# 3dlg-hcvc/tricolo

Measured on AMD Instinct MI355X. Metric: trimodal training samples/sec (32^3 voxel + 6-view), higher is better.
Workload: dtype f16 (f16 activation storage + f16 MFMA operands, fp32 accumulate; bf16x3 heads/GRU; within 1e-3 of the fp32 reference)

## Files before the change

tricolo_amd/csrc/bn_pool.hip:

```cpp
#include "common.h"
#include "../../include/tricolo_hip.h"

__global__ void bn_finalize_kernel(const float* __restrict__ partial, int ntiles, int C, const int* __restrict__ count_dev,
                                   int count_host, const float* __restrict__ gamma, const float* __restrict__ beta,
                                   float* running_mean, float* running_var, long long* num_batches_tracked, float momentum,
                                   float eps, float* __restrict__ mean_out, float* __restrict__ invstd_out,
                                   float* __restrict__ scale_out, float* __restrict__ shift_out) {
    __shared__ double ssum[4], ssq[4];
    const int c = blockIdx.x;
    float pg = 0.f, pb = 0.f, prm = 0.f, prv = 0.f;
    int pcount = count_host;
    if (threadIdx.x == 0) {
        pg = gamma[c]; pb = beta[c];
        if (running_mean) { prm = running_mean[c]; prv = running_var[c]; }
        if (count_dev) pcount = *count_dev;
    }
    double s = 0.0, q = 0.0;
#pragma unroll 8
    for (int tIdx = threadIdx.x; tIdx < ntiles; tIdx += 256) {
        s += (double)partial[((size_t)tIdx * 2 + 0) * C + c];
        q += (double)partial[((size_t)tIdx * 2 + 1) * C + c];
    }
#pragma unroll
    for (int o = 32; o > 0; o >>= 1) { s += __shfl_xor(s, o); q += __shfl_xor(q, o); }
// ... 691 lines not shown
    const int tc = threadIdx.x % tpr, tr = threadIdx.x / tpr;
    const int n = *row_count;
    for (int cc = 0; cc < cpt; ++cc) {
        const int c4 = tc + cc * tpr;
        float4 sg = make_float4(0, 0, 0, 0), sgy = make_float4(0, 0, 0, 0);
        if (c4 < C4 && tr < rpp)
#pragma unroll 4
            for (int i = blockIdx.x * rpp + tr; i < n; i += gridDim.x * rpp) {
                const long r = row_pos[i];
                const float4 gv = Act<T>::ld4(g + r * C + c4 * 4), yv = Act<T>::ld4(y + r * C + c4 * 4);
                sg.x += gv.x; sg.y += gv.y; sg.z += gv.z; sg.w += gv.w;
                sgy.x += gv.x * yv.x; sgy.y += gv.y * yv.y; sgy.z += gv.z * yv.z; sgy.w += gv.w * yv.w;
            }
        __syncthreads();
        if (c4 < C4 && tr < rpp) {
            float* p = sh + ((size_t)tr * tpr + tc) * 8;
            p[0] = sg.x; p[1] = sg.y; p[2] = sg.z; p[3] = sg.w; p[4] = sgy.x; p[5] = sgy.y; p[6] = sgy.z; p[7] = sgy.w;
        }
        __syncthreads();
        if (tr == 0 && c4 < C4) {
            float a[8] = {0, 0, 0, 0, 0, 0, 0, 0};
            for (int rr = 0; rr < rpp; ++rr) {
                const float* p = sh + ((size_t)rr * tpr + tc) * 8;
#pragma unroll
                for (int k = 0; k < 8; ++k) a[k] += p[k];
            }
            float* o = partial + (size_t)blockIdx.x * 2 * C;
#pragma unroll
            for (int k = 0; k < 4; ++k) { o[c4 * 4 + k] = a[k]; o[C + c4 * 4 + k] = a[4 + k]; }
        }
    }
}
template <typename T>
__global__ void bn_bwd_apply_rows_kernel(const T* __restrict__ y, const T* g, const float4* __restrict__ c1, const float4* __restrict__ c2,
                                         const float4* __restrict__ c3, T* dy, int C4, const int* __restrict__ row_pos,
                                         const int* __restrict__ row_count) {
    const long total = (long)(*row_count) * C4;
    for (long i = (long)blockIdx.x * blockDim.x + threadIdx.x; i < total; i += (long)gridDim.x * blockDim.x) {
        const int c = (int)(i % C4);
        const long o = ((long)row_pos[i / C4] * C4 + c) * 4;
        const float4 yv = Act<T>::ld4(y + o), gv = Act<T>::ld4(g + o), a = c1[c], b = c2[c], d = c3[c];
        Act<T>::st4(dy + o, make_float4(a.x * gv.x + b.x + d.x * yv.x, a.y * gv.y + b.y + d.y * yv.y, a.z * gv.z + b.z + d.z * yv.z,
                                        a.w * gv.w + b.w + d.w * yv.w));
    }
}
extern "C" size_t tri_bn_bwd_rows_scratch(int C) { return (size_t)BNR_BLOCKS * 2 * C * sizeof(float) + 3 * (size_t)C * sizeof(float); }
extern "C" int tri_bn_bwd_rows(const void* y, const void* g, int C, const int* row_pos, const int* row_count, long max_rows, const float* gamma,
                               const float* mean, const float* invstd, void* dy, float* dgamma, float* dbeta, float out_scale, void* scratch,
                               int act_fmt, void* stream) {
    if (C % 4 || !row_pos || !row_count || !scratch) { tri_set_error("tri_bn_bwd_rows: C % 4, row list and scratch required"); return TRI_ERR_ARG; }
    hipStream_t st = (hipStream_t)stream;
    float* partial = (float*)scratch;
    float* co = partial + (size_t)BNR_BLOCKS * 2 * C;
    const int C4 = C / 4, tpr = C4 < 256 ? C4 : 256, rpp = 256 / tpr;
    const size_t smem = (size_t)rpp * tpr * 8 * sizeof(float);
    TRI_ACT_DISPATCH(act_fmt, bn_bwd_reduce_rows_kernel<T><<<BNR_BLOCKS, 256, smem, st>>>((const T*)y, (const T*)g, C, row_pos, row_count, partial));
    bn_bwd_finalize_kernel<<<C, 256, 0, st>>>(partial, BNR_BLOCKS, C, row_count, 0, gamma, mean, invstd, dgamma, dbeta, co, co + C, co + 2 * C, out_scale);
    const int grid = ew_grid(max_rows * C4 / 4 + 1);
    TRI_ACT_DISPATCH(act_fmt, bn_bwd_apply_rows_kernel<T><<<grid, 256, 0, st>>>((const T*)y, (const T*)g, (const float4*)co, (const float4*)(co + C),
                                                                                 (const float4*)(co + 2 * C), (T*)dy, C4, row_pos, row_count));
    return tri_check_launch("tri_bn_bwd_rows");
}

extern "C" int tri_bn_bwd_apply_rows(const void* y, const void* g, const float* c1, const float* c2, const float* c3, void* dy, int C,
                                     const int* row_pos, const int* row_count, long max_rows, int act_fmt, void* stream) {
    if (C % 4 || !row_pos || !row_count) { tri_set_error("tri_bn_bwd_apply_rows: C % 4 and a row list required"); return TRI_ERR_ARG; }
    const int C4 = C / 4, grid = ew_grid(max_rows * C4 / 4 + 1);
    TRI_ACT_DISPATCH(act_fmt, bn_bwd_apply_rows_kernel<T><<<grid, 256, 0, (hipStream_t)stream>>>((const T*)y, (const T*)g, (const float4*)c1,
        (const float4*)c2, (const float4*)c3, (T*)dy, C4, row_pos, row_count));
    return tri_check_launch("tri_bn_bwd_apply_rows");
}

template <typename T>
__global__ __launch_bounds__(256) void pool3d_bwd_route_reduce_kernel(const T* __restrict__ y, const float4* __restrict__ scale,
                                                                      const float4* __restrict__ shift, const uint8_t* __restrict__ mask,
                                                                      const T* __restrict__ pooled, const T* __restrict__ dpooled, int B, int D,
                                                                      int C4, T* __restrict__ g, float* __restrict__ partial) {
    __shared__ float sh[256][8];
    const int Do = D >> 1;
    const long total = (long)B * Do * Do * Do * C4;
    const int c = threadIdx.x % C4;
    const float4 s = scale[c], t = shift[c];
    float4 sg = make_float4(0.f, 0.f, 0.f, 0.f), sgy = sg;
    for (unsigned i = blockIdx.x * blockDim.x + threadIdx.x; i < (unsigned)total; i += gridDim.x * blockDim.x) {
        const PoolWin w = pool_window(mask, i / (unsigned)C4, (unsigned)D);
        if (!w.bits) continue;
        const float4 pm = Act<T>::ld4(pooled + (size_t)i * 4), dp = Act<T>::ld4(dpooled + (size_t)i * 4);
        route_window<T>(y, s, t, w, (unsigned)D, (unsigned)C4, (unsigned)c, pm, dp, g, sg, sgy);
    }
    float* p = sh[threadIdx.x];
    p[0] = sg.x; p[1] = sg.y; p[2] = sg.z; p[3] = sg.w; p[4] = sgy.x; p[5] = sgy.y; p[6] = sgy.z; p[7] = sgy.w;
    __syncthreads();
    if ((int)threadIdx.x < C4) {
        float a[8] = {0, 0, 0, 0, 0, 0, 0, 0};
        for (int r = threadIdx.x; r < 256; r += C4)
#pragma unroll
            for (int k = 0; k < 8; ++k) a[k] += sh[r][k];
        float* o = partial + (size_t)blockIdx.x * 2 * C4 * 4;
#pragma unroll
        for (int k = 0; k < 4; ++k) { o[c * 4 + k] = a[k]; o[C4 * 4 + c * 4 + k] = a[4 + k]; }
    }
}
extern "C" int tri_pool3d_bwd_route_reduce_num_blocks(int B, int D, int C) {
    return ew_grid((long)B * (D / 2) * (D / 2) * (D / 2) * (C / 4));
}
extern "C" int tri_pool3d_bwd_route_reduce(const void* y, const float* scale, const float* shift, const uint8_t* mask, const void* pooled,
                                           const void* dpooled, int B, int D, int C, void* g, float* partial, int act_fmt, void* stream) {
    if (C % 4 || C / 4 > 256 || 256 % (C / 4)) { tri_set_error("tri_pool3d_bwd_route_reduce: C / 4 must divide 256"); return TRI_ERR_ARG; }
    if (!pool_args_ok("tri_pool3d_bwd_route_reduce", mask, B, D, C)) return TRI_ERR_ARG;
    const int nblk = tri_pool3d_bwd_route_reduce_num_blocks(B, D, C);
    TRI_ACT_DISPATCH(act_fmt, pool3d_bwd_route_reduce_kernel<T><<<nblk, 256, 0, (hipStream_t)stream>>>(
        (const T*)y, (const float4*)scale, (const float4*)shift, mask, (const T*)pooled, (const T*)dpooled, B, D, C / 4, (T*)g, partial));
    return tri_check_launch("tri_pool3d_bwd_route_reduce");
}

template <typename T>
__global__ void maxpool2d_fwd_kernel(const T* __restrict__ x, int N, int H, int W, int C4, T* __restrict__ out,
                                     uchar4* __restrict__ arg, const float4* __restrict__ scale, const float4* __restrict__ shift) {
    const int Ho = (H + 1) / 2, Wo = (W + 1) / 2;
    const long total = (long)N * Ho * Wo * C4;
    for (long i = (long)blockIdx.x * blockDim.x + threadIdx.x; i < total; i += (long)gridDim.x * blockDim.x) {
        int c = (int)(i % C4);
        long pos = i / C4;
        int ow = (int)(pos % Wo); long r = pos / Wo;
        int oh = (int)(r % Ho); int n = (int)(r / Ho);
        float4 best = make_float4(-INFINITY, -INFINITY, -INFINITY, -INFINITY);
        uchar4 bi = make_uchar4(0, 0, 0, 0);
        float4 s4 = make_float4(1.f, 1.f, 1.f, 1.f), b4 = make_float4(0.f, 0.f, 0.f, 0.f);
        if (scale) { s4 = scale[c]; b4 = shift[c]; }
#pragma unroll
        for (int kh = 0; kh < 3; ++kh) {
            int ih = oh * 2 - 1 + kh;
            if ((unsigned)ih >= (unsigned)H) continue;
#pragma unroll
            for (int kw = 0; kw < 3; ++kw) {
                int iw = ow * 2 - 1 + kw;
                if ((unsigned)iw >= (unsigned)W) continue;
                float4 v = Act<T>::ld4(x + ((((long)n * H + ih) * W + iw) * C4 + c) * 4);
                if (scale) {
                    v.x = fmaxf(__fmaf_rn(v.x, s4.x, b4.x), 0.f); v.y = fmaxf(__fmaf_rn(v.y, s4.y, b4.y), 0.f);
                    v.z = fmaxf(__fmaf_rn(v.z, s4.z, b4.z), 0.f); v.w = fmaxf(__fmaf_rn(v.w, s4.w, b4.w), 0.f);
                }
                unsigned char k = (unsigned char)(kh * 3 + kw);
                if (v.x > best.x) { best.x = v.x; bi.x = k; }
                if (v.y > best.y) { best.y = v.y; bi.y = k; }
                if (v.z > best.z) { best.z = v.z; bi.z = k; }
                if (v.w > best.w) { best.w = v.w; bi.w = k; }
            }
        }
        Act<T>::st4(out + i * 4, best);
        if (arg) arg[i] = bi;
    }
}
template <typename T>
__global__ __launch_bounds__(256) void maxpool2d_fwd8_kernel(const T* __restrict__ x, int N, int H, int W, int C8, T* __restrict__ out,
                                                             uint2* __restrict__ arg, const float* __restrict__ scale, const float* __restrict__ shift) {
    const int Ho = (H + 1) / 2, Wo = (W + 1) / 2;
    constexpr int G = 4;
    const int Hg = (Ho + G - 1) / G;
    const long total = (long)N * Hg * Wo * C8;
    for (long i = (long)blockIdx.x * blockDim.x + threadIdx.x; i < total; i += (long)gridDim.x * blockDim.x) {
        const int c = (int)(i % C8);
        long pos = i / C8;
        const int ow = (int)(pos % Wo); long r = pos / Wo;
        const int og = (int)(r % Hg); const int n = (int)(r / Hg);
        float s8[8], b8[8];
#pragma unroll
        for (int k = 0; k < 8; ++k) { s8[k] = 1.f; b8[k] = 0.f; }
        if (scale) {
#pragma unroll
            for (int k = 0; k < 8; ++k) { s8[k] = scale[c * 8 + k]; b8[k] = shift[c * 8 + k]; }
        }
        bool okw[3];
#pragma unroll
        for (int kw = 0; kw < 3; ++kw) okw[kw] = (unsigned)(ow * 2 - 1 + kw) < (unsigned)W;
        auto load_row = [&](int ih, uint4 (&d)[3]) {
#pragma unroll
            for (int kw = 0; kw < 3; ++kw) {
                d[kw] = make_uint4(0u, 0u, 0u, 0u);
                if ((unsigned)ih < (unsigned)H && okw[kw]) d[kw] = *(const uint4*)(x + ((((long)n * H + ih) * W + ow * 2 - 1 + kw) * C8 + c) * 8);
            }
        };
        uint4 row0[3], row1[3], row2[3];
        const int oh0 = og * G;
        load_row(oh0 * 2 - 1, row0);
#pragma unroll
        for (int g = 0; g < G; ++g) {
            const int oh = oh0 + g;
            if (oh >= Ho) break;
            load_row(oh * 2, row1);
            load_row(oh * 2 + 1, row2);
            float best[8];
            unsigned bi[8];
#pragma unroll
            for (int k = 0; k < 8; ++k) { best[k] = -INFINITY; bi[k] = 0u; }
#pragma unroll
            for (int kh = 0; kh < 3; ++kh) {
                if ((unsigned)(oh * 2 - 1 + kh) >= (unsigned)H) continue;
#pragma unroll
                for (int kw = 0; kw < 3; ++kw) {
                    if (!okw[kw]) continue;
                    const uint4 q = kh == 0 ? row0[kw] : (kh == 1 ? row1[kw] : row2[kw]);
#pragma unroll
                    for (int k = 0; k < 8; ++k) {
                        float e = (float)((const T*)&q)[k];
                        if (scale) e = fmaxf(__fmaf_rn(e, s8[k], b8[k]), 0.f);
                        if (e > best[k]) { best[k] = e; bi[k] = (unsigned)(kh * 3 + kw); }
                    }
                }
            }
            uint4 o;
            T* op = (T*)&o;
#pragma unroll
            for (int k = 0; k < 8; ++k) op[k] = (T)best[k];
            const long oi = (((long)n * Ho + oh) * Wo + ow) * C8 + c;
            *(uint4*)(out + oi * 8) = o;
            if (arg) arg[oi] = make_uint2(bi[0] | (bi[1] << 8) | (bi[2] << 16) | (bi[3] << 24), bi[4] | (bi[5] << 8) | (bi[6] << 16) | (bi[7] << 24));
#pragma unroll
            for (int kw = 0; kw < 3; ++kw) row0[kw] = row2[kw];
        }
    }
}
extern "C" int tri_maxpool2d_fwd(const void* x, int N, int H, int W, int C, void* out, uint8_t* arg, const float* bn_scale,
                                 const float* bn_shift, int act_fmt, void* stream) {
    static int pool8 = -1;
    if (pool8 < 0) pool8 = 1;
    if (pool8 && act_fmt != TRI_FMT_F32 && C % 8 == 0) {
        const long total8 = (long)N * (((H + 1) / 2 + 3) / 4) * ((W + 1) / 2) * (C / 8);
        if (act_fmt == TRI_FMT_F16)
            maxpool2d_fwd8_kernel<f16_t><<<ew_grid(total8), 256, 0, (hipStream_t)stream>>>((const f16_t*)x, N, H, W, C / 8, (f16_t*)out, (uint2*)arg, bn_scale, bn_shift);
        else
            maxpool2d_fwd8_kernel<bf16_t><<<ew_grid(total8), 256, 0, (hipStream_t)stream>>>((const bf16_t*)x, N, H, W, C / 8, (bf16_t*)out, (uint2*)arg, bn_scale, bn_shift);
        return tri_check_launch("tri_maxpool2d_fwd");
    }
    long total = (long)N * ((H + 1) / 2) * ((W + 1) / 2) * (C / 4);
    TRI_ACT_DISPATCH(act_fmt, maxpool2d_fwd_kernel<T><<<ew_grid(total), 256, 0, (hipStream_t)stream>>>((const T*)x, N, H, W, C / 4, (T*)out, (uchar4*)arg,
                                                                                                  (const float4*)bn_scale, (const float4*)bn_shift));
    return tri_check_launch("tri_maxpool2d_fwd");
}

template <typename T>
__global__ void maxpool2d_bwd_kernel(const uchar4* __restrict__ arg, const T* __restrict__ dout, int N, int H, int W, int C4,
                                     T* __restrict__ dx) {
    const int Ho = (H + 1) / 2, Wo = (W + 1) / 2;
    const long total = (long)N * H * W * C4;
    for (long i = (long)blockIdx.x * blockDim.x + threadIdx.x; i < total; i += (long)gridDim.x * blockDim.x) {
        int c = (int)(i % C4);
        long pos = i / C4;
        int w = (int)(pos % W); long r = pos / W;
        int h = (int)(r % H); int n = (int)(r / H);
        float4 acc = make_float4(0.f, 0.f, 0.f, 0.f);
        for (int oh = h / 2; oh <= (h + 1) / 2; ++oh) {
            if (oh >= Ho) continue;
            for (int ow = w / 2; ow <= (w + 1) / 2; ++ow) {
                if (ow >= Wo) continue;
                unsigned char me = (unsigned char)((h - (oh * 2 - 1)) * 3 + (w - (ow * 2 - 1)));
                long o = (((long)n * Ho + oh) * Wo + ow) * C4 + c;
                uchar4 a = arg[o];
                float4 d = Act<T>::ld4(dout + o * 4);
                if (a.x == me) acc.x += d.x;
                if (a.y == me) acc.y += d.y;
                if (a.z == me) acc.z += d.z;
                if (a.w == me) acc.w += d.w;
            }
        }
        Act<T>::st4(dx + i * 4, acc);
    }
}
template <typename T>
__global__ void maxpool2d_bwd2x2_kernel(const uchar4* __restrict__ arg, const T* __restrict__ dout, int N, int H, int W, int C4,
                                        T* __restrict__ dx) {
    const int Ho = H / 2, Wo = W / 2;
    const long total = (long)N * Ho * Wo * C4;
    for (long i = (long)blockIdx.x * blockDim.x + threadIdx.x; i < total; i += (long)gridDim.x * blockDim.x) {
        const int c = (int)(i % C4);
        long pos = i / C4;
        const int bw = (int)(pos % Wo); long r = pos / Wo;
        const int bh = (int)(r % Ho); const int n = (int)(r / Ho);
        uchar4 a[2][2];
        float4 d[2][2];
#pragma unroll
        for (int u = 0; u < 2; ++u)
#pragma unroll
            for (int v = 0; v < 2; ++v) {
                a[u][v] = make_uchar4(255, 255, 255, 255);
                d[u][v] = make_float4(0.f, 0.f, 0.f, 0.f);
                if (bh + u < Ho && bw + v < Wo) {
                    const long o = (((long)n * Ho + bh + u) * Wo + bw + v) * C4 + c;
                    a[u][v] = arg[o];
                    d[u][v] = Act<T>::ld4(dout + o * 4);
                }
            }
#define TRI_PICK(A, D, TAP) make_float4(A.x == TAP ? D.x : 0.f, A.y == TAP ? D.y : 0.f, A.z == TAP ? D.z : 0.f, A.w == TAP ? D.w : 0.f)
#define TRI_ADD4(P, Q) make_float4(P.x + Q.x, P.y + Q.y, P.z + Q.z, P.w + Q.w)
        const float4 p00 = TRI_PICK(a[0][0], d[0][0], 4);
        const float4 p01 = TRI_ADD4(TRI_PICK(a[0][0], d[0][0], 5), TRI_PICK(a[0][1], d[0][1], 3));
        const float4 p10 = TRI_ADD4(TRI_PICK(a[0][0], d[0][0], 7), TRI_PICK(a[1][0], d[1][0], 1));
        float4 p11 = TRI_ADD4(TRI_PICK(a[0][0], d[0][0], 8), TRI_PICK(a[0][1], d[0][1], 6));
        const float4 p11b = TRI_ADD4(TRI_PICK(a[1][0], d[1][0], 2), TRI_PICK(a[1][1], d[1][1], 0));
        p11 = TRI_ADD4(p11, p11b);
#undef TRI_PICK
#undef TRI_ADD4
        T* o = dx + ((((long)n * H + 2 * bh) * W + 2 * bw) * C4 + c) * 4;
        Act<T>::st4(o, p00);
        Act<T>::st4(o + (long)C4 * 4, p01);
        Act<T>::st4(o + (long)W * C4 * 4, p10);
        Act<T>::st4(o + ((long)W + 1) * C4 * 4, p11);
    }
}
extern "C" int tri_maxpool2d_bwd(const uint8_t* arg, const void* dout, int N, int H, int W, int C, void* dx, int act_fmt, void* stream) {
    if (H % 2 == 0 && W % 2 == 0) {
        long total = (long)N * (H / 2) * (W / 2) * (C / 4);
        TRI_ACT_DISPATCH(act_fmt, maxpool2d_bwd2x2_kernel<T><<<ew_grid(total), 256, 0, (hipStream_t)stream>>>((const uchar4*)arg, (const T*)dout, N, H, W, C / 4, (T*)dx));
        return tri_check_launch("tri_maxpool2d_bwd");
    }
    long total = (long)N * H * W * (C / 4);
    TRI_ACT_DISPATCH(act_fmt, maxpool2d_bwd_kernel<T><<<ew_grid(total), 256, 0, (hipStream_t)stream>>>((const uchar4*)arg, (const T*)dout, N, H, W, C / 4, (T*)dx));
    return tri_check_launch("tri_maxpool2d_bwd");
}

template <typename T>
__device__ __forceinline__ void stem_route_2x2(const uchar4* __restrict__ arg, const T* __restrict__ dpool, int n, int bh, int bw, int Ho,
                                               int Wo, int C4, int c, float4 g[4]) {
    uchar4 a[2][2];
    float4 d[2][2];
#pragma unroll
    for (int u = 0; u < 2; ++u)
#pragma unroll
        for (int v = 0; v < 2; ++v) {
            a[u][v] = make_uchar4(255, 255, 255, 255);
            d[u][v] = make_float4(0.f, 0.f, 0.f, 0.f);
            if (bh + u < Ho && bw + v < Wo) {
                const long o = (((long)n * Ho + bh + u) * Wo + bw + v) * C4 + c;
                a[u][v] = arg[o];
                d[u][v] = Act<T>::ld4(dpool + o * 4);
            }
        }
#define TRI_PICK(A, D, TAP) make_float4(A.x == TAP ? D.x : 0.f, A.y == TAP ? D.y : 0.f, A.z == TAP ? D.z : 0.f, A.w == TAP ? D.w : 0.f)
#define TRI_ADD4(P, Q) make_float4(P.x + Q.x, P.y + Q.y, P.z + Q.z, P.w + Q.w)
    g[0] = TRI_PICK(a[0][0], d[0][0], 4);
    g[1] = TRI_ADD4(TRI_PICK(a[0][0], d[0][0], 5), TRI_PICK(a[0][1], d[0][1], 3));
    g[2] = TRI_ADD4(TRI_PICK(a[0][0], d[0][0], 7), TRI_PICK(a[1][0], d[1][0], 1));
    const float4 p = TRI_ADD4(TRI_PICK(a[0][0], d[0][0], 8), TRI_PICK(a[0][1], d[0][1], 6));
    const float4 q = TRI_ADD4(TRI_PICK(a[1][0], d[1][0], 2), TRI_PICK(a[1][1], d[1][1], 0));
    g[3] = TRI_ADD4(p, q);
#undef TRI_PICK
#undef TRI_ADD4
}
template <typename T>
__device__ __forceinline__ float4 rnd4(float4 v) { return make_float4(Act<T>::rnd(v.x), Act<T>::rnd(v.y), Act<T>::rnd(v.z), Act<T>::rnd(v.w)); }

static int stem_blocks_per_wg() {
    static int v = -1;
    if (v < 0) v = 64;
    return v;
}
template <typename T>
__global__ __launch_bounds__(256) void stem_bwd_reduce8_kernel(const T* __restrict__ y, const uint8_t* __restrict__ arg, const T* __restrict__ dpool,
                                                               int N, int H, int W, int C, float* __restrict__ partial,
                                                               const float* __restrict__ rs, const float* __restrict__ rb, int STEM_BLOCKS_PER_WG) {
    extern __shared__ float sh[];
    const int C8 = C >> 3, Ho = H >> 1, Wo = W >> 1;
    const int tpr = C8 < 256 ? C8 : 256, rpp = 256 / tpr;
    const int tc = threadIdx.x % tpr, tr = threadIdx.x / tpr;
    const long nb = (long)N * Ho * Wo;
    const long r0 = (long)blockIdx.x * STEM_BLOCKS_PER_WG, r1 = r0 + STEM_BLOCKS_PER_WG < nb ? r0 + STEM_BLOCKS_PER_WG : nb;
    float sg[8], sgy[8];
#pragma unroll
    for (int k = 0; k < 8; ++k) { sg[k] = 0.f; sgy[k] = 0.f; }
    if (tc < C8 && tr < rpp) {
        float s8[8], b8[8];
#pragma unroll
        for (int k = 0; k < 8; ++k) { s8[k] = rs[tc * 8 + k]; b8[k] = rb[tc * 8 + k]; }
#pragma unroll 2
        for (long r = r0 + tr; r < r1; r += rpp) {
            const int bw = (int)(r % Wo); const long q = r / Wo;
            const int bh = (int)(q % Ho), n = (int)(q / Ho);
            uint4 yr[4], dr[2][2];
            uint2 ar[2][2];
#pragma unroll
            for (int k = 0; k < 4; ++k) yr[k] = *(const uint4*)(y + ((((long)n * H + 2 * bh + (k >> 1)) * W + 2 * bw + (k & 1)) * C + tc * 8));
#pragma unroll
            for (int u = 0; u < 2; ++u)
#pragma unroll
                for (int v = 0; v < 2; ++v) {
// ... 344 lines not shown
```

tricolo_amd/csrc/conv_igemm.hip:

```cpp
#include "common.h"
#include <stdlib.h>
#include <map>
#include <mutex>
#include "../../include/tricolo_hip.h"
#include "conv_vox.h"

struct ConvArgs {
    const void* in;
    const void* w_hi;
    const void* w_lo;
    void* out;
    const uint8_t* row_mask;
    const int* row_pos;
    const int* row_count;
    const float* bias;
    float* stats;
    float* slab;
    int B, ID, IH, IW, Cin;
    int OD, OH, OW, Cout;
    int KD, KH, KW, stride, pd, ph, pw;
    int transposed, act, accumulate;
    int Kpad, M, ntaps, cin_shift, ksplit, steps_per_split;
    unsigned in_bytes;
    int nunits;
// ... 1415 lines not shown
        const int nxt = tile + gridDim.x;
        if (nxt < sg.ntiles && !(p.h_abl & 8)) fetch(nxt);
        const char* sb = smem + buf * slab_bytes;
        const int img = tile / sg.tiles_per_img, oh0 = (tile - img * sg.tiles_per_img) * sg.TH;
        f32x4 acc[NPT][4];
#pragma unroll
        for (int j = 0; j < NPT; ++j)
#pragma unroll
            for (int ct = 0; ct < 4; ++ct) acc[j][ct] = (f32x4){0.f, 0.f, 0.f, 0.f};
        if (!(p.h_abl & 1))
#pragma unroll
        for (int kh = 0; kh < KH; ++kh) {
            v8 b[NPT];
#pragma unroll
            for (int j = 0; j < NPT; ++j) b[j] = *(const v8*)(sb + boff[j] + kh * sg.row_bytes);
#pragma unroll
            for (int j = 0; j < NPT; ++j)
#pragma unroll
                for (int ct = 0; ct < 4; ++ct) acc[j][ct] = MM::mma(wf[kh][ct], b[j], acc[j][ct]);
        }
        AT* const obase = (AT*)p.out + ((size_t)img * OH + oh0) * OW * p.Cout;
#pragma unroll
        for (int j = 0; j < NPT; ++j) {
            if (inside[j] && oh0 + orow[j] < OH) {
                AT* o = obase + ooff[j];
#pragma unroll
                for (int ct = 0; ct < 4; ++ct) {
                    f32x4 v = acc[j][ct];
                    if (!(p.h_abl & 4)) Act<AT>::st4(o + ct * 16, make_float4(v[0], v[1], v[2], v[3]));
                    if (p.stats) {
                        v[0] = Act<AT>::rnd(v[0]); v[1] = Act<AT>::rnd(v[1]); v[2] = Act<AT>::rnd(v[2]); v[3] = Act<AT>::rnd(v[3]);
                        cs[ct] += v;
                        cq[ct] += v * v;
                    }
                }
            }
        }
        if (nxt < sg.ntiles) stash(buf ^ 1);
        __syncthreads();
        buf ^= 1;
    }
    if (p.stats) {
#pragma unroll
        for (int ct = 0; ct < 4; ++ct)
#pragma unroll
            for (int r = 0; r < 4; ++r) {
                float s_ = cs[ct][r], q_ = cq[ct][r];
                s_ += row_ror<8>(s_); q_ += row_ror<8>(q_);
                s_ += row_ror<4>(s_); q_ += row_ror<4>(q_);
                s_ += row_ror<2>(s_); q_ += row_ror<2>(q_);
                s_ += row_ror<1>(s_); q_ += row_ror<1>(q_);
                if (fr == 0) {
                    const int col = ct * 16 + fq * 4 + r;
                    red[(wave * 64 + col) * 2 + 0] = s_;
                    red[(wave * 64 + col) * 2 + 1] = q_;
                }
            }
        __syncthreads();
        if (t < 64) {
            float s_ = 0.f, q_ = 0.f;
#pragma unroll
            for (int w = 0; w < 4; ++w) { s_ += red[(w * 64 + t) * 2]; q_ += red[(w * 64 + t) * 2 + 1]; }
            p.stats[((size_t)blockIdx.x * 2 + 0) * p.Cout + t] = s_;
            p.stats[((size_t)blockIdx.x * 2 + 1) * p.Cout + t] = q_;
        }
    }
}

template <typename AT>
__global__ __launch_bounds__(256) void conv_splitk_finish_kernel(const ConvArgs p) {
    __shared__ float red[16][64][2];
    const int t = threadIdx.x, tc = t & 15, rl = t >> 4;
    const int chunk = blockIdx.x, m0 = chunk * 32, n = blockIdx.y * 64 + tc * 4;
    float4 s4 = make_float4(0.f, 0.f, 0.f, 0.f), q4 = s4;
    const float4 bv = p.bias ? *(const float4*)(p.bias + n) : make_float4(0.f, 0.f, 0.f, 0.f);
    const int Meff = p.row_count ? min(*p.row_count, p.M) : p.M;
#pragma unroll
    for (int rr = 0; rr < 2; ++rr) {
        int m = m0 + rl * 2 + rr;
        if (m >= Meff) continue;
        const size_t pos = p.row_pos ? (size_t)p.row_pos[m] : (size_t)m;
        bool live = p.row_mask ? (p.row_mask[pos] != 0) : true;
        float4 v = make_float4(0.f, 0.f, 0.f, 0.f);
        if (live) {
            const float* sp = p.slab + (size_t)m * p.Cout + n;
            const size_t zs = (size_t)p.M * p.Cout;
            int z = 0;
            for (; z + 4 <= p.ksplit; z += 4) {
                const float4 x0 = *(const float4*)(sp + (size_t)z * zs), x1 = *(const float4*)(sp + (size_t)(z + 1) * zs);
                const float4 x2 = *(const float4*)(sp + (size_t)(z + 2) * zs), x3 = *(const float4*)(sp + (size_t)(z + 3) * zs);
                v.x += x0.x; v.y += x0.y; v.z += x0.z; v.w += x0.w;
                v.x += x1.x; v.y += x1.y; v.z += x1.z; v.w += x1.w;
                v.x += x2.x; v.y += x2.y; v.z += x2.z; v.w += x2.w;
                v.x += x3.x; v.y += x3.y; v.z += x3.z; v.w += x3.w;
            }
            for (; z < p.ksplit; ++z) {
                const float4 x = *(const float4*)(sp + (size_t)z * zs);
                v.x += x.x; v.y += x.y; v.z += x.z; v.w += x.w;
            }
            v.x += bv.x; v.y += bv.y; v.z += bv.z; v.w += bv.w;
            if (p.act == 1) { v.x = fmaxf(v.x, 0.f); v.y = fmaxf(v.y, 0.f); v.z = fmaxf(v.z, 0.f); v.w = fmaxf(v.w, 0.f); }
            else if (p.act == 2) { v.x = tanhf(v.x); v.y = tanhf(v.y); v.z = tanhf(v.z); v.w = tanhf(v.w); }
        }
        AT* o = (AT*)p.out + pos * p.Cout + n;
        if (p.accumulate) { float4 e = Act<AT>::ld4(o); v.x += e.x; v.y += e.y; v.z += e.z; v.w += e.w; }
        Act<AT>::st4(o, v);
        if (sizeof(AT) == 2) v = make_float4(Act<AT>::rnd(v.x), Act<AT>::rnd(v.y), Act<AT>::rnd(v.z), Act<AT>::rnd(v.w));
        s4.x += v.x; s4.y += v.y; s4.z += v.z; s4.w += v.w;
        q4.x += v.x * v.x; q4.y += v.y * v.y; q4.z += v.z * v.z; q4.w += v.w * v.w;
    }
    if (p.stats) {
        float* d = &red[rl][tc * 4][0];
        d[0] = s4.x; d[1] = q4.x; d[2] = s4.y; d[3] = q4.y; d[4] = s4.z; d[5] = q4.z; d[6] = s4.w; d[7] = q4.w;
        __syncthreads();
        if (t < 64) {
            float s = 0.f, q = 0.f;
#pragma unroll
            for (int w = 0; w < 16; ++w) { s += red[w][t][0]; q += red[w][t][1]; }
            p.stats[((size_t)chunk * 2 + 0) * p.Cout + blockIdx.y * 64 + t] = s;
            p.stats[((size_t)chunk * 2 + 1) * p.Cout + blockIdx.y * 64 + t] = q;
        }
    }
}

__device__ __forceinline__ void prep_store(bool f16, uint16_t* hi, bf16_t* lo, size_t idx, float v) {
    if (f16) { hi[idx] = __builtin_bit_cast(uint16_t, (f16_t)v); return; }
    const bf16_t h = (bf16_t)v;
    hi[idx] = __builtin_bit_cast(uint16_t, h);
    if (lo) lo[idx] = (bf16_t)(v - (float)h);
}

__device__ __forceinline__ size_t prep_index(bool frag, int row, int k, int kpad) {
    if (!frag) return (size_t)row * kpad + k;
    return ((size_t)(row >> 4) * (kpad >> 5) + (k >> 5)) * 512 + ((((k & 31) >> 3) * 16 + (row & 15)) << 3) + (k & 7);
}

__device__ __forceinline__ void prep_store4(bool f16, uint16_t* hi, bf16_t* lo, size_t idx, float4 v) {
    if (f16) {
        f16x4 h;
        h[0] = (f16_t)v.x; h[1] = (f16_t)v.y; h[2] = (f16_t)v.z; h[3] = (f16_t)v.w;
        *(f16x4*)(hi + idx) = h;
        return;
    }
    bf16x4 h;
    h[0] = (bf16_t)v.x; h[1] = (bf16_t)v.y; h[2] = (bf16_t)v.z; h[3] = (bf16_t)v.w;
    *(bf16x4*)(hi + idx) = h;
    if (lo) {
        bf16x4 l;
        l[0] = (bf16_t)(v.x - (float)h[0]); l[1] = (bf16_t)(v.y - (float)h[1]); l[2] = (bf16_t)(v.z - (float)h[2]); l[3] = (bf16_t)(v.w - (float)h[3]);
        *(bf16x4*)(lo + idx) = l;
    }
}

__global__ void weight_prep_kernel(const float* __restrict__ w, long s_row, long s_tap, long s_inner, int rows, int ntaps,
                                   int inner, int inner_pad, int Kpad, uint16_t* __restrict__ hi, bf16_t* __restrict__ lo, int f16, int frag) {
    long idx = (long)blockIdx.x * blockDim.x + threadIdx.x;
    long total = (long)rows * Kpad;
    if (idx >= total) return;
    int row = (int)(idx / Kpad), k = (int)(idx - (long)row * Kpad);
    int tap = k / inner_pad, i = k - tap * inner_pad;
    float v = 0.f;
    if (tap < ntaps && i < inner) v = w[row * s_row + tap * s_tap + i * s_inner];
    prep_store(f16 != 0, hi, lo, prep_index(frag != 0, row, k, Kpad), v);
}

__global__ __launch_bounds__(256) void weight_prep_multi_kernel(const TriPrepDesc* __restrict__ descs) {
    __shared__ float tile[64 * 73];
    const TriPrepDesc d = descs[blockIdx.y];
    uint16_t* hi = (uint16_t*)d.hi;
    bf16_t* lo = (bf16_t*)d.lo;
    const bool f16 = d.fmt == TRI_FMT_F16, frag = d.frag != 0;
    const int t = threadIdx.x, nt = d.ntaps;
    const long span = (long)d.inner * nt;
    if (nt > 1 && d.s_tap == 1 && d.s_inner == nt && d.s_row == span && span <= 64 * 73 && d.inner == d.inner_pad) {
        const bool vec = (span & 3) == 0 && (d.inner_pad & 3) == 0 && (d.kpad & 3) == 0 && (((uintptr_t)d.w) & 15) == 0;
        for (int row = blockIdx.x; row < d.rows; row += gridDim.x) {
            const float* src = d.w + (size_t)row * d.s_row;
            if (vec) {
                for (int e = t * 4; e < span; e += 1024) *(float4*)(tile + e) = *(const float4*)(src + e);
                __syncthreads();
                for (int k = t * 4; k < d.kpad; k += 1024) {
                    const int tap = k / d.inner_pad, i = k - tap * d.inner_pad;
                    float4 v = make_float4(0.f, 0.f, 0.f, 0.f);
                    if (tap < nt) v = make_float4(tile[i * nt + tap], tile[(i + 1) * nt + tap], tile[(i + 2) * nt + tap], tile[(i + 3) * nt + tap]);
                    prep_store4(f16, hi, lo, prep_index(frag, row, k, d.kpad), v);
                }
            } else {
                for (int e = t; e < span; e += 256) tile[e] = src[e];
                __syncthreads();
                for (int k = t; k < d.kpad; k += 256) {
                    const int tap = k / d.inner_pad, i = k - tap * d.inner_pad;
                    prep_store(f16, hi, lo, prep_index(frag, row, k, d.kpad), tap < nt ? tile[i * nt + tap] : 0.f);
                }
            }
            __syncthreads();
        }
        return;
    }
    if (d.s_inner == 1 && d.s_tap == d.inner && d.s_row == span && d.inner == d.inner_pad && (span & 3) == 0 && (d.kpad & 3) == 0 &&
        (((uintptr_t)d.w) & 15) == 0) {
        const unsigned q4 = (unsigned)(d.kpad >> 2), total4 = (unsigned)d.rows * q4, used = (unsigned)span;
        for (unsigned e = blockIdx.x * 256u + t; e < total4; e += gridDim.x * 256u) {
            const unsigned row = e / q4, k = (e - row * q4) * 4u;
            float4 v = make_float4(0.f, 0.f, 0.f, 0.f);
            if (k < used) v = *(const float4*)(d.w + (size_t)row * span + k);
            prep_store4(f16, hi, lo, prep_index(frag, (int)row, (int)k, d.kpad), v);
        }
        return;
    }
    const bool torch_t = nt > 1 && nt <= 9 && d.s_tap == 1 && d.s_row == nt && d.s_inner == (long)d.rows * nt;
    const bool plane_t = d.s_row == 1 && d.s_tap == d.rows && d.s_inner == (long)d.rows * nt;
    if ((torch_t || plane_t) && d.inner == d.inner_pad) {
        const int RT = torch_t ? 8 : 32;
        const int run = torch_t ? RT * nt : RT, ld = run + 1;
        const int planes = torch_t ? 1 : nt;
        const int rtiles = (d.rows + RT - 1) / RT, itiles = (d.inner + 63) / 64;
        const long ntile = (long)rtiles * itiles * planes;
        for (long tl = blockIdx.x; tl < ntile; tl += gridDim.x) {
            const int plane = (int)(tl / ((long)rtiles * itiles));
            const int rem = (int)(tl - (long)plane * rtiles * itiles);
            const int r0 = (rem / itiles) * RT, i0 = (rem % itiles) * 64;
            const int rows_here = min(RT, d.rows - r0);
            const int run_here = torch_t ? rows_here * nt : rows_here;
            for (int e = t; e < 64 * run; e += 256) {
                const int il = e / run, r = e - il * run;
                float v = 0.f;
                if (i0 + il < d.inner && r < run_here)
                    v = d.w[(size_t)(i0 + il) * d.s_inner + (torch_t ? (size_t)r0 * nt + r : (size_t)plane * d.s_tap + r0 + r)];
                tile[il * ld + r] = v;
            }
            __syncthreads();
            if ((d.inner & 3) == 0 && (d.inner_pad & 3) == 0 && (d.kpad & 3) == 0) {
                for (int e = t; e < 16 * run; e += 256) {
                    const int il = (e & 15) * 4, r = e >> 4;
                    const int row_l = torch_t ? r / nt : r, tap = torch_t ? r - row_l * nt : plane;
                    if (row_l < rows_here && i0 + il < d.inner)
                        prep_store4(f16, hi, lo, prep_index(frag, r0 + row_l, tap * d.inner_pad + i0 + il, d.kpad),
                                    make_float4(tile[il * ld + r], tile[(il + 1) * ld + r], tile[(il + 2) * ld + r], tile[(il + 3) * ld + r]));
                }
            } else
            for (int e = t; e < 64 * run; e += 256) {
                const int il = e & 63, r = e >> 6;
                const int row_l = torch_t ? r / nt : r, tap = torch_t ? r - row_l * nt : plane;
                if (row_l < rows_here && i0 + il < d.inner)
                    prep_store(f16, hi, lo, prep_index(frag, r0 + row_l, tap * d.inner_pad + i0 + il, d.kpad), tile[il * ld + r]);
            }
            __syncthreads();
        }
        const int kused = nt * d.inner_pad, padw = d.kpad - kused;
        if (padw > 0)
            for (long e = (long)blockIdx.x * 256 + t; e < (long)d.rows * padw; e += (long)gridDim.x * 256) {
                const int row = (int)(e / padw), k = kused + (int)(e - (long)row * padw);
                prep_store(f16, hi, lo, prep_index(frag, row, k, d.kpad), 0.f);
            }
        return;
    }
    const long total = (long)d.rows * d.kpad;
    for (long idx = (long)blockIdx.x * blockDim.x + threadIdx.x; idx < total; idx += (long)gridDim.x * blockDim.x) {
        int row = (int)(idx / d.kpad), k = (int)(idx - (long)row * d.kpad);
        int tap = k / d.inner_pad, i = k - tap * d.inner_pad;
        float v = 0.f;
        if (tap < d.ntaps && i < d.inner) v = d.w[row * d.s_row + tap * d.s_tap + i * d.s_inner];
        prep_store(f16, hi, lo, prep_index(frag, row, k, d.kpad), v);
    }
}

extern "C" int tri_weight_prep_multi(const TriPrepDesc* descs_dev, int n, void* stream) {
    if (n <= 0) return TRI_OK;
    static int gx = 0;
    if (!gx) gx = 512;
    weight_prep_multi_kernel<<<dim3(gx, n), 256, 0, (hipStream_t)stream>>>(descs_dev);
    return tri_check_launch("tri_weight_prep_multi");
}

extern "C" int tri_weight_prep(const float* w, long s_row, long s_tap, long s_inner, int rows, int ntaps, int inner,
                               int inner_pad, void* w_hi, void* w_lo, int fmt, int frag, void* stream) {
    if (fmt == TRI_FMT_F16 && w_lo) { tri_set_error("tri_weight_prep: the f16 operand format has no lo part"); return TRI_ERR_ARG; }
    if (inner_pad % 4 != 0 || inner > inner_pad) { tri_set_error("tri_weight_prep: inner_pad must be a multiple of 4 >= inner"); return TRI_ERR_ARG; }
    if (frag && rows % 16 != 0) { tri_set_error("tri_weight_prep: the fragment-major order needs rows % 16 == 0"); return TRI_ERR_ARG; }
    int Kpad = (ntaps * inner_pad + 31) / 32 * 32;
    long total = (long)rows * Kpad;
    int blocks = (int)((total + 255) / 256);
    weight_prep_kernel<<<blocks, 256, 0, (hipStream_t)stream>>>(w, s_row, s_tap, s_inner, rows, ntaps, inner, inner_pad, Kpad,
                                                                (uint16_t*)w_hi, (bf16_t*)w_lo, fmt == TRI_FMT_F16 ? 1 : 0, frag ? 1 : 0);
    return tri_check_launch("tri_weight_prep");
}


static int ilog2_exact(int v) {
    for (int s = 0; s < 31; ++s) if ((1 << s) == v) return s;
    return -1;
}

template <int BN, int NSPLIT, typename AT>
static int launch_conv(const ConvArgs& a, hipStream_t stream) {
    constexpr int STAGE = NSPLIT * (128 * 64 + BN * 64);
    constexpr int WAVES_M = (BN >= 64) ? 2 : 4;
    size_t smem = 2 * STAGE + 512 + WAVES_M * BN * 2 * sizeof(float);
    static bool attr_set = false;
    if (!attr_set) {
        hipFuncSetAttribute((const void*)conv_igemm_kernel<BN, NSPLIT, AT>, hipFuncAttributeMaxDynamicSharedMemorySize, (int)smem);
        attr_set = true;
    }
    int mt = (a.M + 127) / 128, nt = a.Cout / BN;
    conv_igemm_kernel<BN, NSPLIT, AT><<<dim3(mt * nt, a.ksplit), 256, smem, stream>>>(a);
    int rc = tri_check_launch("tri_conv");
    if (rc || a.ksplit == 1) return rc;
    conv_splitk_finish_kernel<AT><<<dim3((a.M + 31) / 32, a.Cout / 64), 256, 0, stream>>>(a);
    return tri_check_launch("tri_conv_splitk_finish");
}

static int conv_bn(int cout) { return cout % 128 == 0 ? 128 : (cout % 64 == 0 ? 64 : 32); }

struct ConvPlan {
    int bn;
    int halo;
    int h_tr, h_rows, h_slab_bytes, h_nr, h_mtiles, h_dbuf;
    int h_v5;
    int h_grid;
    int h_wgrec;
    int stem;
    int stem_grid;
    int vox0;
    int vox0_grid;
    int voxb, voxb_grid;
    int s2g, s2g_units;
    int voxg;
    int voxg_units, voxg_ct, voxg_spu;
    int c64;
    int c64_grid;
    int s2d;
    int pw, pw_tr;
    int dma;
    int nunits;
    int ksplit, per_split;
};

static int conv_target_blocks() {
    static int v = -1;
    if (v < 0) v = 0;
    return v;
}

static bool halo_disabled() {
    static int v = -1;
    if (v < 0) { const char* e = getenv("TRICOLO_NO_HALO"); v = (e && e[0] == '1') ? 1 : 0; }
    return v == 1;
}

static int num_cus() {
    static int v = 0;
    if (!v) {
        int dev = 0;
        hipDeviceProp_t pr;
        if (hipGetDevice(&dev) == hipSuccess && hipGetDeviceProperties(&pr, dev) == hipSuccess && pr.multiProcessorCount > 0) v = pr.multiProcessorCount;
        else v = 256;
    }
    return v;
}

int tri_internal_num_cus() { return num_cus(); }

static bool halo_geometry(int B, int H, int W, int cin, int cout, int TM, ConvPlan* pl) {
    const int BM = 64 * TM, P = W + 2;
    if (W > BM) return false;
    const int TR = BM / W;
    int k;
    if (H % TR == 0) k = 1;
    else if (TR % H == 0) k = TR / H;
    else return false;
    const int rows = TR + 2 * k;
    const int slab = ((rows * P + 1) * 128 + 4095) / 4096 * 4096;
    if (slab / 4096 > 10) return false;
    (void)cout;
    pl->halo = TM; pl->h_tr = TR; pl->h_rows = rows; pl->h_slab_bytes = slab; pl->h_nr = 3; pl->h_dbuf = 0;
    pl->h_mtiles = (B * H + TR - 1) / TR;
    {
        const int NT = cout / 64, items = pl->h_mtiles * NT;
        const size_t smem = (size_t)slab + (size_t)HALO_NR * 8192 + 2048;
        int per_cu = (int)(163840 / (smem + 256));
        per_cu = per_cu < 1 ? 1 : (per_cu > 3 ? 3 : per_cu);
        int slots = num_cus() * per_cu / NT * NT;
        if (slots < NT) slots = NT;
        pl->h_grid = items < slots ? items : slots;
        pl->h_wgrec = items >= 4 * slots ? 1 : 0;
        static int rows_kernel = -1;
        if (rows_kernel < 0) { const char* e = getenv("TRICOLO_HALO_ROWS"); rows_kernel = e ? atoi(e) : 1; }
        pl->h_v5 = 0;
        int g = num_cus() / NT * NT;
        if (g < NT) g = NT;
        static int half_tiles = -1;
        if (half_tiles < 0) half_tiles = 3;
        static int deep = -1;
        if (deep < 0) deep = 1;
        if (rows_kernel && (cin == 64 || (deep && cin >= 256) || 2 * items <= half_tiles * g || rows_kernel == 2) && (TM == 2 || (TM == 3 && cin != 64)) &&
            2 * (size_t)slab + 3 * (size_t)HROWS_SLOT + 8192 <= 163840) {
            pl->h_v5 = 1;
            pl->h_grid = items < g ? items : g;
            pl->h_wgrec = 1;
        }
    }
    return true;
}

static bool stem_disabled() {
    static int v = -1;
    if (v < 0) { const char* e = getenv("TRICOLO_NO_STEM"); v = (e && e[0] == '1') ? 1 : 0; }
    return v == 1;
}
static bool stem_geometry(int B, int IH, int IW, int cin, int OH, int OW, int cout, int KD, int KH, int KW, int stride, int pd, int ph, int pw,
                          StemGeom* g) {
    if (KD != 1 || pd != 0 || cin != 4 || stride != 2 || cout != 64 || (KH != 3 && KH != 5 && KH != 7) || KW > 8 || OW % 16 || IW % 2) return false;
    if (pw < 0 || ph < 0 || IW + pw > 2 * OW + 6 || (long)B * IH * IW * 8 >= ((long)1 << 31)) return false;
    const int per_row = OW / 16;
    static int npt = -1;
    if (npt < 0) npt = 2;
    if (per_row > 4 * npt) return false;
    int TH = 4 * npt / per_row;
    if (TH > OH) TH = OH;
    g->npt = npt;
    g->TH = TH;
    g->slab_rows = (TH - 1) * 2 + KH;
    g->row_bytes = (OW + 3) * 16;
// ... 590 lines not shown
```

Baseline: 13530.

## Restructure maxpool8 row reduction and add vectorized double-buffered weight-prep paths

The 8-wide maxpool forward kernel now uses 32-bit index math and clamped branchless loads. It reduces each input row once and carries the shared boundary row's max and argmax to the next output row instead of keeping the raw data. The weight-prep multi kernel gains vectorized fast paths for the transposed and plane layouts: it prefetches the next tile into registers while the current tile goes through shared memory, then writes 8 f16/bf16 values at a time. These changes aim to cut global-memory transactions and scalar work in the per-step pooling and weight conversion. The new paths add complex index bookkeeping and raise register and shared-memory pressure.

```diff
diff --git a/tricolo_amd/csrc/bn_pool.hip b/tricolo_amd/csrc/bn_pool.hip
--- a/tricolo_amd/csrc/bn_pool.hip
+++ b/tricolo_amd/csrc/bn_pool.hip
@@ -867,63 +867,93 @@
         if (arg) arg[i] = bi;
     }
 }
-template <typename T>
-__global__ __launch_bounds__(256) void maxpool2d_fwd8_kernel(const T* __restrict__ x, int N, int H, int W, int C8, T* __restrict__ out,
+#ifndef POOL8_WAVES
+#define POOL8_WAVES 6
+#endif
+#ifndef POOL8_ROWS
+#define POOL8_ROWS 4
+#endif
+template <typename T>
+__global__ __launch_bounds__(256, POOL8_WAVES) void maxpool2d_fwd8_kernel(const T* __restrict__ x, int N, int H, int W, int C8, T* __restrict__ out,
                                                              uint2* __restrict__ arg, const float* __restrict__ scale, const float* __restrict__ shift) {
     const int Ho = (H + 1) / 2, Wo = (W + 1) / 2;
-    constexpr int G = 4;
+    constexpr int G = POOL8_ROWS;
     const int Hg = (Ho + G - 1) / G;
-    const long total = (long)N * Hg * Wo * C8;
-    for (long i = (long)blockIdx.x * blockDim.x + threadIdx.x; i < total; i += (long)gridDim.x * blockDim.x) {
-        const int c = (int)(i % C8);
-        long pos = i / C8;
-        const int ow = (int)(pos % Wo); long r = pos / Wo;
-        const int og = (int)(r % Hg); const int n = (int)(r / Hg);
+    const unsigned total = (unsigned)N * Hg * Wo * C8;
+    for (unsigned i = blockIdx.x * blockDim.x + threadIdx.x; i < total; i += gridDim.x * blockDim.x) {
+        const int c = (int)(i % (unsigned)C8);
+        unsigned pos = i / (unsigned)C8;
+        const int ow = (int)(pos % (unsigned)Wo); unsigned r = pos / (unsigned)Wo;
+        const int og = (int)(r % (unsigned)Hg); const int n = (int)(r / (unsigned)Hg);
         float s8[8], b8[8];
 #pragma unroll
         for (int k = 0; k < 8; ++k) { s8[k] = 1.f; b8[k] = 0.f; }
         if (scale) {
-#pragma unroll
-            for (int k = 0; k < 8; ++k) { s8[k] = scale[c * 8 + k]; b8[k] = shift[c * 8 + k]; }
+            const float4 sa = ((const float4*)scale)[c * 2], sb = ((const float4*)scale)[c * 2 + 1];
+            const float4 ba = ((const float4*)shift)[c * 2], bb = ((const float4*)shift)[c * 2 + 1];
+            s8[0] = sa.x; s8[1] = sa.y; s8[2] = sa.z; s8[3] = sa.w; s8[4] = sb.x; s8[5] = sb.y; s8[6] = sb.z; s8[7] = sb.w;
+            b8[0] = ba.x; b8[1] = ba.y; b8[2] = ba.z; b8[3] = ba.w; b8[4] = bb.x; b8[5] = bb.y; b8[6] = bb.z; b8[7] = bb.w;
         }
         bool okw[3];
-#pragma unroll
-        for (int kw = 0; kw < 3; ++kw) okw[kw] = (unsigned)(ow * 2 - 1 + kw) < (unsigned)W;
+        int iwc[3];
+#pragma unroll
+        for (int kw = 0; kw < 3; ++kw) {
+            okw[kw] = (unsigned)(ow * 2 - 1 + kw) < (unsigned)W;
+            iwc[kw] = min(max(ow * 2 - 1 + kw, 0), W - 1);
+        }
         auto load_row = [&](int ih, uint4 (&d)[3]) {
+            const int ihc = min(max(ih, 0), H - 1);
+#pragma unroll
+            for (int kw = 0; kw < 3; ++kw) d[kw] = *(const uint4*)(x + ((((long)n * H + ihc) * W + iwc[kw]) * C8 + c) * 8);
+        };
+        auto reduce_row = [&](int ih, const uint4 (&d)[3], unsigned base, float (&m)[8]) -> unsigned {
+            unsigned id[8];
+#pragma unroll
+            for (int k = 0; k < 8; ++k) { m[k] = -INFINITY; id[k] = 0u; }
+            const bool okh = (unsigned)ih < (unsigned)H;
 #pragma unroll
             for (int kw = 0; kw < 3; ++kw) {
-                d[kw] = make_uint4(0u, 0u, 0u, 0u);
-                if ((unsigned)ih < (unsigned)H && okw[kw]) d[kw] = *(const uint4*)(x + ((((long)n * H + ih) * W + ow * 2 - 1 + kw) * C8 + c) * 8);
-            }
+                const bool ok = okh & okw[kw];
+#pragma unroll
+                for (int k = 0; k < 8; ++k) {
+                    float e = (float)((const T*)&d[kw])[k];
+                    if (scale) e = fmaxf(__fmaf_rn(e, s8[k], b8[k]), 0.f);
+                    const bool gt = ok & (e > m[k]);
+                    m[k] = gt ? e : m[k];
+                    id[k] = gt ? base + (unsigned)kw : id[k];
+                }
+            }
+            unsigned p = id[0];
+#pragma unroll
+            for (int k = 1; k < 8; ++k) p |= id[k] << (4 * k);
+            return p;
         };
-        uint4 row0[3], row1[3], row2[3];
         const int oh0 = og * G;
-        load_row(oh0 * 2 - 1, row0);
-#pragma unroll
+        float m0[8];
+        unsigned p0;
+        {
+            uint4 raw[3];
+            load_row(oh0 * 2 - 1, raw);
+            p0 = reduce_row(oh0 * 2 - 1, raw, 0u, m0);
+        }
+#pragma unroll 1
         for (int g = 0; g < G; ++g) {
             const int oh = oh0 + g;
             if (oh >= Ho) break;
-            load_row(oh * 2, row1);
-            load_row(oh * 2 + 1, row2);
-            float best[8];
+            uint4 raw1[3], raw2[3];
+            load_row(oh * 2, raw1);
+            load_row(oh * 2 + 1, raw2);
+            float best[8], m[8];
             unsigned bi[8];
 #pragma unroll
-            for (int k = 0; k < 8; ++k) { best[k] = -INFINITY; bi[k] = 0u; }
-#pragma unroll
-            for (int kh = 0; kh < 3; ++kh) {
-                if ((unsigned)(oh * 2 - 1 + kh) >= (unsigned)H) continue;
-#pragma unroll
-                for (int kw = 0; kw < 3; ++kw) {
-                    if (!okw[kw]) continue;
-                    const uint4 q = kh == 0 ? row0[kw] : (kh == 1 ? row1[kw] : row2[kw]);
-#pragma unroll
-                    for (int k = 0; k < 8; ++k) {
-                        float e = (float)((const T*)&q)[k];
-                        if (scale) e = fmaxf(__fmaf_rn(e, s8[k], b8[k]), 0.f);
-                        if (e > best[k]) { best[k] = e; bi[k] = (unsigned)(kh * 3 + kw); }
-                    }
-                }
-            }
+            for (int k = 0; k < 8; ++k) { best[k] = m0[k]; bi[k] = (p0 >> (4 * k)) & 15u; }
+            const unsigned p1 = reduce_row(oh * 2, raw1, 3u, m);
+#pragma unroll
+            for (int k = 0; k < 8; ++k) if (m[k] > best[k]) { best[k] = m[k]; bi[k] = (p1 >> (4 * k)) & 15u; }
+            p0 = reduce_row(oh * 2 + 1, raw2, 0u, m0);
+            const unsigned p2 = p0 + 0x66666666u;
+#pragma unroll
+            for (int k = 0; k < 8; ++k) if (m0[k] > best[k]) { best[k] = m0[k]; bi[k] = (p2 >> (4 * k)) & 15u; }
             uint4 o;
             T* op = (T*)&o;
 #pragma unroll
@@ -931,8 +961,6 @@
             const long oi = (((long)n * Ho + oh) * Wo + ow) * C8 + c;
             *(uint4*)(out + oi * 8) = o;
             if (arg) arg[oi] = make_uint2(bi[0] | (bi[1] << 8) | (bi[2] << 16) | (bi[3] << 24), bi[4] | (bi[5] << 8) | (bi[6] << 16) | (bi[7] << 24));
-#pragma unroll
-            for (int kw = 0; kw < 3; ++kw) row0[kw] = row2[kw];
         }
     }
 }
@@ -940,12 +968,12 @@
                                  const float* bn_shift, int act_fmt, void* stream) {
     static int pool8 = -1;
     if (pool8 < 0) pool8 = 1;
-    if (pool8 && act_fmt != TRI_FMT_F32 && C % 8 == 0) {
-        const long total8 = (long)N * (((H + 1) / 2 + 3) / 4) * ((W + 1) / 2) * (C / 8);
+    const long rows8 = (long)N * (((H + 1) / 2 + POOL8_ROWS - 1) / POOL8_ROWS) * ((W + 1) / 2) * (C / 8);
+    if (pool8 && act_fmt != TRI_FMT_F32 && C % 8 == 0 && rows8 < (1l << 31)) {
         if (act_fmt == TRI_FMT_F16)
-            maxpool2d_fwd8_kernel<f16_t><<<ew_grid(total8), 256, 0, (hipStream_t)stream>>>((const f16_t*)x, N, H, W, C / 8, (f16_t*)out, (uint2*)arg, bn_scale, bn_shift);
+            maxpool2d_fwd8_kernel<f16_t><<<ew_grid(rows8), 256, 0, (hipStream_t)stream>>>((const f16_t*)x, N, H, W, C / 8, (f16_t*)out, (uint2*)arg, bn_scale, bn_shift);
         else
-            maxpool2d_fwd8_kernel<bf16_t><<<ew_grid(total8), 256, 0, (hipStream_t)stream>>>((const bf16_t*)x, N, H, W, C / 8, (bf16_t*)out, (uint2*)arg, bn_scale, bn_shift);
+            maxpool2d_fwd8_kernel<bf16_t><<<ew_grid(rows8), 256, 0, (hipStream_t)stream>>>((const bf16_t*)x, N, H, W, C / 8, (bf16_t*)out, (uint2*)arg, bn_scale, bn_shift);
         return tri_check_launch("tri_maxpool2d_fwd");
     }
     long total = (long)N * ((H + 1) / 2) * ((W + 1) / 2) * (C / 4);
diff --git a/tricolo_amd/csrc/conv_igemm.hip b/tricolo_amd/csrc/conv_igemm.hip
--- a/tricolo_amd/csrc/conv_igemm.hip
+++ b/tricolo_amd/csrc/conv_igemm.hip
@@ -1591,6 +1591,26 @@
     }
 }
 
+__device__ __forceinline__ void prep_store8(bool f16, uint16_t* hi, bf16_t* lo, size_t idx, const float (&v)[8]) {
+    if (f16) {
+        f16x8 h;
+#pragma unroll
+        for (int j = 0; j < 8; ++j) h[j] = (f16_t)v[j];
+        *(f16x8*)(hi + idx) = h;
+        return;
+    }
+    bf16x8 h;
+#pragma unroll
+    for (int j = 0; j < 8; ++j) h[j] = (bf16_t)v[j];
+    *(bf16x8*)(hi + idx) = h;
+    if (lo) {
+        bf16x8 l;
+#pragma unroll
+        for (int j = 0; j < 8; ++j) l[j] = (bf16_t)(v[j] - (float)h[j]);
+        *(bf16x8*)(lo + idx) = l;
+    }
+}
+
 __global__ void weight_prep_kernel(const float* __restrict__ w, long s_row, long s_tap, long s_inner, int rows, int ntaps,
                                    int inner, int inner_pad, int Kpad, uint16_t* __restrict__ hi, bf16_t* __restrict__ lo, int f16, int frag) {
     long idx = (long)blockIdx.x * blockDim.x + threadIdx.x;
@@ -1603,8 +1623,12 @@
     prep_store(f16 != 0, hi, lo, prep_index(frag != 0, row, k, Kpad), v);
 }
 
-__global__ __launch_bounds__(256) void weight_prep_multi_kernel(const TriPrepDesc* __restrict__ descs) {
-    __shared__ float tile[64 * 73];
+#ifndef PREP_GRID
+#define PREP_GRID 512
+#endif
+#define PREP_ROW 4644
+__global__ __launch_bounds__(256, 4) void weight_prep_multi_kernel(const TriPrepDesc* __restrict__ descs) {
+    __shared__ __attribute__((aligned(16))) float tile[2 * PREP_ROW];
     const TriPrepDesc d = descs[blockIdx.y];
     uint16_t* hi = (uint16_t*)d.hi;
     bf16_t* lo = (bf16_t*)d.lo;
@@ -1613,6 +1637,56 @@
     const long span = (long)d.inner * nt;
     if (nt > 1 && d.s_tap == 1 && d.s_inner == nt && d.s_row == span && span <= 64 * 73 && d.inner == d.inner_pad) {
         const bool vec = (span & 3) == 0 && (d.inner_pad & 3) == 0 && (d.kpad & 3) == 0 && (((uintptr_t)d.w) & 15) == 0;
+        const int ldf = d.inner + 4;
+        if (vec && (d.inner & 7) == 0 && (d.kpad & 7) == 0 && nt < 1024 && (long)nt * ldf <= PREP_ROW) {
+            int wr[5], rd[3];
+#pragma unroll
+            for (int p = 0; p < 5; ++p) {
+                const int e = (t + 256 * p) * 4, ci = e / nt, tap = e - ci * nt;
+                wr[p] = e < span ? (((tap * ldf + ci) << 10) | tap) : -1;
+            }
+#pragma unroll
+            for (int p = 0; p < 3; ++p) {
+                const int k = (t + 256 * p) * 8, tap = k / d.inner_pad, i = k - tap * d.inner_pad;
+                rd[p] = k < d.kpad ? (tap < nt ? tap * ldf + i : -1) : -2;
+            }
+            float4 v[5];
+            auto load_row = [&](int row) {
+                const float* src = d.w + (size_t)row * d.s_row;
+#pragma unroll
+                for (int p = 0; p < 5; ++p) if (wr[p] >= 0) v[p] = *(const float4*)(src + (t + 256 * p) * 4);
+            };
+            int row = blockIdx.x, cur = 0;
+            if (row < d.rows) load_row(row);
+            for (; row < d.rows; row += gridDim.x) {
+                float* b = tile + cur * PREP_ROW;
+#pragma unroll
+                for (int p = 0; p < 5; ++p) {
+                    if (wr[p] < 0) continue;
+                    int a = wr[p] >> 10, tap = wr[p] & 1023;
+                    const float e4[4] = {v[p].x, v[p].y, v[p].z, v[p].w};
+#pragma unroll
+                    for (int j = 0; j < 4; ++j) {
+                        b[a] = e4[j];
+                        if (++tap == nt) { tap = 0; a -= (nt - 1) * ldf - 1; } else a += ldf;
+                    }
+                }
+                __syncthreads();
+                if (row + (int)gridDim.x < d.rows) load_row(row + gridDim.x);
+#pragma unroll
+                for (int p = 0; p < 3; ++p) {
+                    if (rd[p] == -2) continue;
+                    float o[8] = {0.f, 0.f, 0.f, 0.f, 0.f, 0.f, 0.f, 0.f};
+                    if (rd[p] >= 0) {
+                        const float4 a = *(const float4*)(b + rd[p]), c = *(const float4*)(b + rd[p] + 4);
+                        o[0] = a.x; o[1] = a.y; o[2] = a.z; o[3] = a.w; o[4] = c.x; o[5] = c.y; o[6] = c.z; o[7] = c.w;
+                    }
+                    prep_store8(f16, hi, lo, prep_index(frag, row, (t + 256 * p) * 8, d.kpad), o);
+                }
+                cur ^= 1;
+            }
+            return;
+        }
         for (int row = blockIdx.x; row < d.rows; row += gridDim.x) {
             const float* src = d.w + (size_t)row * d.s_row;
             if (vec) {
@@ -1648,7 +1722,77 @@
         return;
     }
     const bool torch_t = nt > 1 && nt <= 9 && d.s_tap == 1 && d.s_row == nt && d.s_inner == (long)d.rows * nt;
-    const bool plane_t = d.s_row == 1 && d.s_tap == d.rows && d.s_inner == (long)d.rows * nt;
+    const bool plane_t = d.s_row == 1 && (d.s_tap == d.rows || nt == 1) && d.s_inner == (long)d.rows * nt;
+    if ((torch_t || plane_t) && d.inner == d.inner_pad && (d.inner & 7) == 0 && (d.rows & 3) == 0 && (d.kpad & 7) == 0 &&
+        (((uintptr_t)d.w) & 15) == 0) {
+        const int RT = torch_t ? 16 : 128;
+        const int run = torch_t ? RT * nt : RT, run4 = run >> 2, ld = run + 1;
+        const int planes = torch_t ? 1 : nt;
+        const int rtiles = (d.rows + RT - 1) / RT, itiles = (d.inner + 63) / 64;
+        const int ntile = rtiles * itiles * planes;
+        const int ntx = torch_t ? nt : 1;
+        const int ld_dq = 256 / run4, ld_dr = (256 % run4) * 4;
+        const int il0 = t / run4, rr0 = (t - il0 * run4) * 4;
+        const int st_dq = 32 / ntx, st_dr = 32 % ntx;
+        const int row_l0 = (t >> 3) / ntx, tap0 = (t >> 3) - row_l0 * ntx;
+        float4 v[9];
+        auto load_tile = [&](int tl) {
+            const int plane = tl / (rtiles * itiles), rem = tl - plane * rtiles * itiles;
+            const int r0 = (rem / itiles) * RT, i0 = (rem % itiles) * 64;
+            const int run_here = min(RT, d.rows - r0) * ntx;
+            const float* src = d.w + (torch_t ? (size_t)r0 * nt : (size_t)plane * d.s_tap + r0);
+            int il = il0, r = rr0;
+#pragma unroll
+            for (int p = 0; p < 9; ++p) {
+                if (il < 64 && i0 + il < d.inner && r < run_here) v[p] = *(const float4*)(src + (size_t)(i0 + il) * d.s_inner + r);
+                il += ld_dq; r += ld_dr;
+                if (r >= run) { r -= run; ++il; }
+            }
+        };
+        int tl = blockIdx.x;
+        if (tl < ntile) load_tile(tl);
+        for (; tl < ntile; tl += gridDim.x) {
+            {
+                int il = il0, r = rr0;
+#pragma unroll
+                for (int p = 0; p < 9; ++p) {
+                    if (il < 64) {
+                        float* q = tile + il * ld + r;
+                        q[0] = v[p].x; q[1] = v[p].y; q[2] = v[p].z; q[3] = v[p].w;
+                    }
+                    il += ld_dq; r += ld_dr;
+                    if (r >= run) { r -= run; ++il; }
+                }
+            }
+            __syncthreads();
+            if (tl + (int)gridDim.x < ntile) load_tile(tl + gridDim.x);
+            const int plane = tl / (rtiles * itiles), rem = tl - plane * rtiles * itiles;
+            const int r0 = (rem / itiles) * RT, i0 = (rem % itiles) * 64;
+            const int rows_here = min(RT, d.rows - r0);
+            const int il = (t & 7) * 8;
+            int row_l = row_l0, tap = tap0;
+#pragma unroll
+            for (int p = 0; p < 5; ++p) {
+                if (row_l < rows_here && i0 + il < d.inner) {
+                    const int r = (t >> 3) + 32 * p;
+                    float o[8];
+#pragma unroll
+                    for (int j = 0; j < 8; ++j) o[j] = tile[(il + j) * ld + r];
+                    prep_store8(f16, hi, lo, prep_index(frag, r0 + row_l, (torch_t ? tap : plane) * d.inner_pad + i0 + il, d.kpad), o);
+                }
+                row_l += st_dq; tap += st_dr;
+                if (tap >= ntx) { tap -= ntx; ++row_l; }
+            }
+            __syncthreads();
+        }
+        const int kused = nt * d.inner_pad, padw = d.kpad - kused;
+        if (padw > 0)
+            for (long e = (long)blockIdx.x * 256 + t; e < (long)d.rows * padw; e += (long)gridDim.x * 256) {
+                const int row = (int)(e / padw), k = kused + (int)(e - (long)row * padw);
+                prep_store(f16, hi, lo, prep_index(frag, row, k, d.kpad), 0.f);
+            }
+        return;
+    }
     if ((torch_t || plane_t) && d.inner == d.inner_pad) {
         const int RT = torch_t ? 8 : 32;
         const int run = torch_t ? RT * nt : RT, ld = run + 1;
@@ -1707,7 +1851,7 @@
 extern "C" int tri_weight_prep_multi(const TriPrepDesc* descs_dev, int n, void* stream) {
     if (n <= 0) return TRI_OK;
     static int gx = 0;
-    if (!gx) gx = 512;
+    if (!gx) gx = PREP_GRID;
     weight_prep_multi_kernel<<<dim3(gx, n), 256, 0, (hipStream_t)stream>>>(descs_dev);
     return tri_check_launch("tri_weight_prep_multi");
 }
```

Measured after the change: 13530, median of 2. Within noise of the previous version (-0.0%).
